# kohonda/mppi_playground

Hardware: AMD Instinct MI355X
Metric: sample_steps_per_sec (higher is better)
Workload: dtype f32

## Files before the change

mppi_playground_amd/csrc/mppi_capi.hip:

```cpp
#include <hip/hip_runtime.h>
#include <dlfcn.h>
#include <rccl/rccl.h>

#include <cmath>
#include <cstdio>
#include <cstring>
#include <new>
#include <string>
#include <vector>

#include "../../include/mppi_hip.h"
#include "host_search.hpp"
#include "mppi_kernels.hpp"

using namespace mppi;

static constexpr int FOLD_IN_FINALIZE_MAX_ROWS = 64;

struct MppiSolver {
    MppiConfig cfg{};
    Dims d{};
    int ds = 0, dc = 0;
    float4* noise = nullptr;
    float* costs = nullptr;
    unsigned* min_key = nullptr;
    int min_slot = 0;
    float* x0 = nullptr;
    const float* x0_cur = nullptr;
    float* x0_used = nullptr;
    float* coltab = nullptr;
    bool wide = false, limits_set = true;
    mppi::host::MpoState* mpo_dev = nullptr;
// ... 84 lines not shown
    uint8_t* map_pad = nullptr;
    size_t map_bytes[2] = {0, 0}, map_pad_bytes = 0;
    bool params_set = false;
    ModelCtx ctx{};
    int math_fast = 2;
    int reduce_blocks = 512;
    int reduce_chains = 0;
    int timing = 0;
    std::vector<hipEvent_t> ev_pool[5];
    size_t ev_used[5] = {0, 0, 0, 0, 0};
    int GPW = 8, nchunks = 1, colsp = 128;
    bool summary_valid = false;
    int* live_hint = nullptr;
    int* live_hint_dev = nullptr;
    int fold_mode = 0;
    int lazy_state = 0;
    float* b1 = nullptr;
    float* pending_state_out = nullptr;
    uint32_t pending_serial = 0;
    hipStream_t pending_stream = nullptr;
    hipEvent_t lazy_ev = nullptr;
    uint32_t finalize_serial = 0;
    std::string err;
};

namespace {

int fail(mppi_handle_t h, int code, const std::string& msg) {
    if (h) h->err = msg;
    return code;
// ... 237 lines not shown
    d.row = d.T * md.dc;
    d.R = (d.row + 3) / 4;
    for (int k = 0; k < MPPI_MAX_DIM_CONTROL; ++k) {
        d.u_min[k] = cfg->u_min[k]; d.u_max[k] = cfg->u_max[k]; d.sigma[k] = cfg->sigmas[k];
    }
    h->wide = cfg->model == MPPI_MODEL_GENERIC && md.dc != 1 && md.dc != 2 && md.dc != 4;
    h->GPW = 8;
    const int chg = h->GPW * (BLOCK / WAVE);
    h->nchunks = (d.R + chg - 1) / chg;
    h->colsp = h->nchunks * chg * 4;
    *out = h;
    HIP_TRY(h, hipSetDevice(cfg->device));
    const size_t noise_bytes = (size_t)d.tiles * d.R * 64 * sizeof(float4);
    HIP_TRY(h, hipMalloc(&h->noise, noise_bytes));
    HIP_TRY(h, hipMemset(h->noise, 0, noise_bytes));
    HIP_TRY(h, hipMalloc(&h->costs, sizeof(float) * (size_t)d.N));
    HIP_TRY(h, hipMalloc(&h->min_key, 2 * sizeof(unsigned)));
    HIP_TRY(h, hipMemset(h->min_key, 0xFF, 2 * sizeof(unsigned)));
    const size_t x0_floats = (size_t)std::max(md.ds, MPPI_MAX_DIM_STATE);
    HIP_TRY(h, hipMalloc(&h->x0, sizeof(float) * x0_floats));
    HIP_TRY(h, hipMemset(h->x0, 0, sizeof(float) * x0_floats));
    h->x0_cur = h->x0;
    HIP_TRY(h, hipMalloc(&h->x0_used, sizeof(float) * x0_floats));
    HIP_TRY(h, hipMemset(h->x0_used, 0, sizeof(float) * x0_floats));
    h->gen = GenCtx{(uint32_t)cfg->seed, (uint32_t)(cfg->seed >> 32), 0u};
    d.dc = md.dc;
    HIP_TRY(h, hipMalloc(&h->mean, sizeof(float) * (size_t)d.row));
    HIP_TRY(h, hipMemset(h->mean, 0, sizeof(float) * (size_t)d.row));
    HIP_TRY(h, hipMalloc(&h->mean_used, sizeof(float) * (size_t)d.row));
    HIP_TRY(h, hipMemset(h->mean_used, 0, sizeof(float) * (size_t)d.row));
    HIP_TRY(h, hipMalloc(&h->solve_stats, sizeof(float) * 8));
// ... 133 lines not shown
    CLONE(summary, sizeof(float) * (size_t)(MPPI_SUMMARY_HEAD + d.row));
    CLONE(mpo_dev, sizeof(mppi::host::MpoState));
    CLONE(mpo_temp_dev, sizeof(float));
    CLONE(lbps_dev, sizeof(LbpsDev));
    CLONE(lams_dev, sizeof(float) * 3 * STATS_L);
    CLONE(essps_dev, sizeof(EsspsDev));
    CLONE(lambda_dev, sizeof(float));
    if (src->grid0_dev) {
        if (!dst->grid0_dev) HIP_TRY(dst, hipMalloc(&dst->grid0_dev, sizeof(double) * STATS_L));
        CLONE(grid0_dev, sizeof(double) * STATS_L);
    }
#undef CLONE
    dst->min_slot = src->min_slot; dst->gen = src->gen; dst->tiles_valid = src->tiles_valid; dst->injected = src->injected;
    dst->noise_regen = src->noise_regen; dst->mapping = src->mapping; dst->math_fast = src->math_fast;
    dst->reduce_blocks = src->reduce_blocks; dst->reduce_chains = src->reduce_chains; dst->fold_mode = src->fold_mode;
    dst->fused_mode = src->fused_mode; dst->fused_timeout_ticks = src->fused_timeout_ticks; dst->lbps_grid = src->lbps_grid;
    dst->essps_merge0 = src->essps_merge0;
    dst->auto_rule = src->auto_rule; dst->auto_param = src->auto_param; dst->auto_lo = src->auto_lo; dst->auto_hi = src->auto_hi;
    dst->lbps_lo = src->lbps_lo; dst->lbps_hi = src->lbps_hi; dst->grid0_lo = src->grid0_lo; dst->grid0_hi = src->grid0_hi;
    dst->essps_lo = src->essps_lo; dst->essps_hi = src->essps_hi; dst->essps_range = src->essps_range;
    dst->essps_prev_host = src->essps_prev_host; dst->essps_prev_lo = src->essps_prev_lo; dst->essps_prev_hi = src->essps_prev_hi;
    dst->lambda_dev_valid = src->lambda_dev_valid;
    for (int i = 0; i < 3; ++i) dst->stats_host[8 + STATS_L * 3 + i] = src->stats_host[8 + STATS_L * 3 + i];
    dst->last_reduce_blocks = 0;
    dst->summary_valid = src->summary_valid || src->last_reduce_blocks > 0;
    if (!src->summary_valid && src->last_reduce_blocks > 0) {
        if (int rc = clone_buf(dst, dst->partials, src->partials, sizeof(float) * (size_t)2048 * src->colsp)) return rc;
        if (int rc = clone_buf(dst, dst->heads, src->heads, sizeof(float) * (size_t)2048 * 4)) return rc;
        dst->last_reduce_blocks = src->last_reduce_blocks; dst->summary_valid = false;
    }
// ... 566 lines not shown
    const bool defer = h->lazy_state && state_out && !generic && h->mapping == 0;
    if (h->pending_state_out) { if (int rc = flush_state_seq(h, s)) return rc; }
    {
        StageTimer tm(h, 3, s);
#define CALL_FINALIZE(MODEL, FASTV)                                                                   \
    hipLaunchKernelGGL((finalize_kernel<MODEL, FASTV>), dim3(1), dim3(FIN_BLOCK), shmem, s, summaries_dev, num_shards, \
                       h->partials, h->heads, mk, h->last_reduce_blocks, h->colsp, h->summary, h->live_hint_dev,  \
                       lambda, lam_dev, h->d.row, h->d.T, h->x0_cur, store_mean ? h->mean : (float*)nullptr, action_out,  \
                       defer ? (float*)nullptr : state_out, stats_out, h->solve_stats, sg, p2p, h->ctx,          \
                       defer ? h->b1 : (float*)nullptr, defer ? state_out : (float*)nullptr)
        MPPI_DISPATCH(h, CALL_FINALIZE);
#undef CALL_FINALIZE
    }
    HIP_TRY(h, hipGetLastError());
    ++h->finalize_serial;
    if (defer) { h->pending_state_out = state_out; h->pending_serial = h->finalize_serial; h->pending_stream = s; }
    return MPPI_OK;
}

static int order_behind_pending(mppi_handle_t h, hipStream_t s) {
    if (s == h->pending_stream) return MPPI_OK;
    if (!h->lazy_ev) HIP_TRY(h, hipEventCreateWithFlags(&h->lazy_ev, hipEventDisableTiming));
    HIP_TRY(h, hipEventRecord(h->lazy_ev, h->pending_stream));
    HIP_TRY(h, hipStreamWaitEvent(s, h->lazy_ev, 0));
    return MPPI_OK;
}

static int flush_state_seq(mppi_handle_t h, hipStream_t s) {
    if (!h->pending_state_out) return MPPI_OK;
    float* out = h->pending_state_out;
// ... 132 lines not shown
    HIP_TRY(h, hipGetLastError());
    if (rule != FUSED_RULE_NONE) h->lambda_dev_valid = true;
    h->last_reduce_blocks = 0;
    h->summary_valid = true;
    return MPPI_OK;
}

int mppi_set_auto_lambda(mppi_handle_t h, int rule, double param, double lam_min, double lam_max) {
    if (!h || rule < MPPI_AUTO_NONE || rule > MPPI_AUTO_MPO) return fail(h, MPPI_E_INVALID, "bad temperature rule");
    if ((rule == MPPI_AUTO_ESSPS || rule == MPPI_AUTO_LBPS) && (!(lam_min > 0.0) || !(lam_max > lam_min) || !(param > 0.0)))
        return fail(h, MPPI_E_INVALID, "bad temperature rule arguments");
    h->auto_rule = rule; h->auto_param = param; h->auto_lo = lam_min; h->auto_hi = lam_max;
    return MPPI_OK;
}

int mppi_solve(mppi_handle_t h, const float* x0_dev, uint32_t solve_idx, float lambda, float* action_out_dev,
               float* state_seq_out_dev, float* stats_out_dev, void* stream) {
    if (!h) return MPPI_E_INVALID;
    const bool dev = lambda == MPPI_LAMBDA_DEVICE;
    if (dev && h->auto_rule == MPPI_AUTO_NONE)
        return fail(h, MPPI_E_STATE, "MPPI_LAMBDA_DEVICE: no temperature rule configured (mppi_set_auto_lambda)");
    if (x0_dev) { if (int rc = mppi_bind_state(h, x0_dev)) return rc; }
    if (int rc = mppi_sample(h, solve_idx, stream)) return rc;
    if (fused_applies(h, lambda)) {
        if (int rc = flush_state_seq(h, (hipStream_t)stream)) return rc;
        bool declined = false;
        if (int rc = solve_fused(h, lambda, action_out_dev, state_seq_out_dev, stats_out_dev, (hipStream_t)stream, &declined)) return rc;
        if (!declined) {
            if (h->auto_rule == MPPI_AUTO_MPO) return mppi_mpo_step_device(h, stream);
            return MPPI_OK;
        }
    }
    if (int rc = mppi_rollout_cost(h, stream)) return rc;
    if (dev && h->auto_rule == MPPI_AUTO_ESSPS) {
        if (int rc = mppi_essps_lambda_device(h, h->auto_param, h->auto_lo, h->auto_hi, stream)) return rc;
    } else if (dev && h->auto_rule == MPPI_AUTO_LBPS) {
        if (int rc = h->lbps_grid ? mppi_lbps_lambda_device(h, h->auto_param, h->auto_lo, h->auto_hi, stream)
                                  : mppi_lbps_brent_device(h, h->auto_param, h->auto_lo, h->auto_hi, stream)) return rc;
    }
    if (int rc = mppi_weights_reduce(h, lambda, nullptr, stream)) return rc;
    if (int rc = mppi_finalize(h, nullptr, 1, lambda, 1, action_out_dev, state_seq_out_dev, stats_out_dev, stream)) return rc;
    if (h->auto_rule == MPPI_AUTO_MPO) return mppi_mpo_step_device(h, stream);
    return MPPI_OK;
}

int mppi_set_sg_filter(mppi_handle_t h, const float* coeffs_host, int window, const float* history_host) {
// ... 635 lines not shown
        return MPPI_OK;
    }
    if (k == "fused_rearm") {
        if (h->fused_error) *(volatile int*)h->fused_error = 0;
        return MPPI_OK;
    }
    if (k == "lazy_state_seq") {
        if (value && !h->b1) HIP_TRY(h, hipMalloc(&h->b1, sizeof(float) * ((size_t)h->d.row + MPPI_MAX_DIM_STATE)));
        h->lazy_state = value ? 1 : 0;
        return MPPI_OK;
    }
    if (k == "lbps_search") { h->lbps_grid = value ? 1 : 0; return MPPI_OK; }
    if (k == "search_test_drop_block") { h->brent_drop_block = value ? 1 : 0; return MPPI_OK; }
    if (k == "search_rearm") { if (h->search_error) *(volatile int*)h->search_error = 0; return MPPI_OK; }
    if (k == "essps_merge0") { h->essps_merge0 = value != 0; return MPPI_OK; }
    if (k == "fold_path") { h->fold_mode = (value >= 0 && value <= 2) ? (int)value : 0; return MPPI_OK; }
    if (k == "exchange_p2p") {
        if (value && !h->p2p_connected) return fail(h, MPPI_E_STATE, "exchange_p2p: call mppi_p2p_alloc / mppi_p2p_connect first");
        h->p2p_enabled = value != 0;
        return MPPI_OK;
    }
    if (k == "exchange_comm") {
        if (value && !h->comm) return fail(h, MPPI_E_STATE, "exchange_comm: call mppi_comm_init first");
        h->comm_enabled = value != 0;
        return MPPI_OK;
    }
    if (k == "noise_regen") { h->noise_regen = value ? 1 : 0; h->tiles_valid = h->tiles_valid && h->injected; return MPPI_OK; }
    return fail(h, MPPI_E_INVALID, "unknown option " + k);
}

// ... 37 lines not shown
```

mppi_playground_amd/csrc/mppi_finalize.hpp:

```cpp
#pragma once
#include "mppi_exchange.hpp"
#include "mppi_reduce.hpp"

namespace mppi {

template <int NT>
__device__ __forceinline__ int compact_live_rows(const float* __restrict__ heads, int nblocks,
                                                 unsigned short* __restrict__ s_list, int* __restrict__ s_wcnt) {
    constexpr int NWV = NT / WAVE;
    constexpr int MAXCH = REDUCE_MAX_BLOCKS / NT;
    const int lane = threadIdx.x & 63, wv = threadIdx.x >> 6;
    const int nch = (nblocks + NT - 1) / NT;
    unsigned long long mine = 0ull;
    for (int ch = 0; ch < nch; ++ch) {
        const int bb = ch * NT + threadIdx.x;
        const bool f = bb < nblocks && heads[(int64_t)bb * 4 + 3] != 0.0f;
        const unsigned long long mask = __ballot(f);
        if (f) mine |= 1ull << ch;
        if (lane == 0) s_wcnt[ch * NWV + wv] = __popcll(mask);
    }
    __syncthreads();
    int nlive = 0;
    for (int ch = 0; ch < nch; ++ch) {
        int off = 0;
// ... 179 lines not shown
    }
    if (threadIdx.x == 0) rollout_states_checked<MODEL, FAST>(s_x0, T, ctx, state_out, getu);
}

template <int MODEL, int FAST>
__global__ __launch_bounds__(WAVE) void state_seq_kernel(const float* __restrict__ b1_in, int row, int T,
                                                         float* __restrict__ state_out, ModelCtx ctx) {
    constexpr int DS = ModelT<MODEL, FAST>::DS;
    extern __shared__ __attribute__((aligned(16))) float s_b1[];
    for (int i = threadIdx.x; i < row + DS; i += WAVE) s_b1[i] = b1_in[i];
    __syncthreads();
    batch1_rollout<MODEL, FAST>(ctx, s_b1 + row, s_b1, T, state_out);
}

constexpr int FIN_BLOCK = 1024;
template <int MODEL, int FAST>
__device__ __forceinline__ void finalize_tail(const float* summaries, int num_shards, float lambda, int row, int T,
                                              const float* s_x0, float* s_act, float* s_yp,
                                              float* __restrict__ mean_store, float* __restrict__ action_out,
                                              float* __restrict__ state_out, float* __restrict__ stats_out,
                                              float* __restrict__ stats_keep, const SgFilter& sg, const ModelCtx& ctx,
                                              float* __restrict__ b1_out = nullptr, float* __restrict__ poison_out = nullptr) {
    const int stride = MPPI_SUMMARY_HEAD + row;
    float xmax = -INFINITY, cmin = INFINITY;
    for (int g = 0; g < num_shards; ++g) {
        const float m = summaries[(int64_t)g * stride];
        xmax = fmaxf(xmax, (-m) / lambda);
        cmin = fminf(cmin, m);
    }
    float se = 0.f, se2 = 0.f, sec = 0.f;
    for (int g = 0; g < num_shards; ++g) {
        const float* sm = summaries + (int64_t)g * stride;
        const float f = expf((-sm[0]) / lambda - xmax);
        se = fmaf(f, sm[1], se);
        se2 = fmaf(f * f, sm[2], se2);
        sec = fmaf(f, sm[3], sec);
    }
    for (int cidx = threadIdx.x; cidx < row; cidx += FIN_BLOCK) {
        float a = 0.f;
        for (int g = 0; g < num_shards; ++g) {
            const float* sm = summaries + (int64_t)g * stride;
            const float f = expf((-sm[0]) / lambda - xmax);
            a = fmaf(f, sm[MPPI_SUMMARY_HEAD + cidx], a);
        }
        a = a / se;
        s_act[cidx] = a;
        if (sg.window == 0) {
            if (action_out) action_out[cidx] = a;
            if (mean_store) mean_store[cidx] = a;
        }
    }
    if (threadIdx.x == 0) {
        if (stats_out) { stats_out[0] = cmin; stats_out[1] = se; stats_out[2] = se2; stats_out[3] = sec; }
        stats_keep[0] = cmin; stats_keep[1] = se; stats_keep[2] = se2; stats_keep[3] = sec;
        stats_keep[4] = lambda;
    }
    __syncthreads();
    if (sg.window > 0) {
        const int dcn = row / T, p = sg.window / 2, n = 2 * T - 1;
        for (int idx = threadIdx.x; idx < n * dcn; idx += FIN_BLOCK) {
            const int i = idx / dcn, k = idx - i * dcn;
            s_yp[(p + i) * dcn + k] = i < T - 1 ? sg.history[i * dcn + k] : s_act[(i - (T - 1)) * dcn + k];
        }
        __syncthreads();
        for (int idx = threadIdx.x; idx < p * dcn; idx += FIN_BLOCK) {
            const int j = idx / dcn, k = idx - j * dcn;
            s_yp[(p - 1 - j) * dcn + k] = s_yp[(p + j) * dcn + k];
            s_yp[(p + n + j) * dcn + k] = s_yp[(p + n - 1 - j) * dcn + k];
        }
        __syncthreads();
        float filt = 0.0f;
        const int cidx = threadIdx.x;
        if (cidx < row) {
            const int t = cidx / dcn, k = cidx - t * dcn;
            for (int j = 0; j < sg.window; ++j) filt = filt + s_yp[(T - 1 + t + j) * dcn + k] * sg.coeffs[j];
        }
        __syncthreads();
        if (cidx < row) {
            s_act[cidx] = filt;
            if (action_out) action_out[cidx] = filt;
            if (mean_store) mean_store[cidx] = filt;
        }
        for (int idx = threadIdx.x; idx < (T - 1) * dcn; idx += FIN_BLOCK) {
            const int i = idx / dcn, k = idx - i * dcn;
            sg.history[idx] = i < T - 2 ? s_yp[(p + i + 1) * dcn + k] : 0.0f;
        }
        __syncthreads();
        if (threadIdx.x < dcn && T >= 2) sg.history[(T - 2) * dcn + threadIdx.x] = s_act[threadIdx.x];
        __syncthreads();
    }
    if (b1_out) {
        for (int cidx = threadIdx.x; cidx < row; cidx += FIN_BLOCK) b1_out[cidx] = s_act[cidx];
        if (threadIdx.x < ModelT<MODEL, FAST>::DS) b1_out[row + threadIdx.x] = s_x0[threadIdx.x];
        if (poison_out)
            for (int c = threadIdx.x; c < (T + 1) * ModelT<MODEL, FAST>::DS; c += FIN_BLOCK) poison_out[c] = __uint_as_float(0x7fc00000u);
    }
    if (!state_out) return;
    batch1_rollout<MODEL, FAST>(ctx, s_x0, s_act, T, state_out);
}

template <int MODEL, int FAST>
__global__ __launch_bounds__(FIN_BLOCK) void finalize_kernel(const float* __restrict__ summaries, int num_shards,
                                                             const float* __restrict__ partials,
                                                             const float* __restrict__ heads,
                                                             const unsigned* __restrict__ min_key, int nblocks,
                                                             int colsp, float* __restrict__ summary_out,
                                                             int* __restrict__ nlive_out, float lambda_arg,
                                                             const float* __restrict__ lambda_dev, int row, int T,
                                                             const float* __restrict__ x0,
                                                             float* __restrict__ mean_store,
// ... 80 lines not shown
```

mppi_playground_amd/csrc/mppi_kernels.hpp:

```cpp
#pragma once
#include "mppi_common.hpp"
#include "mppi_sample.hpp"
#include "mppi_rollout.hpp"
#include "mppi_reduce.hpp"
#include "mppi_exchange.hpp"
#include "mppi_finalize.hpp"
#include "mppi_search.hpp"
#include "mppi_fused.hpp"
#include "mppi_topk.hpp"
#include "mppi_env.hpp"
#include "mppi_layout.hpp"
#include "mppi_maps.hpp"
```

mppi_playground_amd/csrc/mppi_rollout.hpp:

```cpp
#pragma once
#include "mppi_sample.hpp"

namespace mppi {

template <int MODEL, int FAST, bool GEN, bool UC, bool VAR = false, bool X0OUT = false>
__device__ __forceinline__ float trajectory_cost(const float4* __restrict__ np, uint64_t gi, const GenCtx& gen,
                                                 const float4* mean4, const float* ktab,
                                                 const float* __restrict__ x0, const Dims& d, const ModelCtx& ctx_in,
                                                 bool& bad) {
    using M = ModelT<MODEL, FAST>;
    using K = typename M::K;
    constexpr int DS = M::DS, DC = M::DC, SPG = 4 / DC;
    ModelCtx ctx = ctx_in;
    if constexpr (FAST != 0 && EntryGeneral<M>::value) M::pin_hot(ctx);
    KeyPins pins{gen.seed_lo, gen.seed_hi, gen.seed_lo + 0x9E3779B9u};
    if (GEN) asm volatile("" : "+v"(pins.k0v), "+v"(pins.k1v), "+v"(pins.k0w));
    float s[DS], pu[DC], pl[DC];
#pragma unroll
    for (int j = 0; j < DS; ++j) s[j] = x0[j];
    if (FAST) {
        if constexpr (EntryGeneral<M>::value) {
            M::enter_any(s);
        } else {
            M::check_state(ctx, s, bad);
// ... 94 lines not shown
        if (bad) {
            bool ignore = false;
            total = trajectory_cost<MODEL, 0, GEN, false>(np, gi, gen, mp, s_ktab, x0, d, ctx, ignore);
        }
    }
    return total;
}

template <int MODEL, int FAST>
__device__ __forceinline__ void batch1_rollout(const ModelCtx& ctx, const float* s_x0, const float* s_act, int T,
                                               float* __restrict__ state_out);

#ifndef MPPI_ROLLOUT_ATTR
#define MPPI_ROLLOUT_ATTR
#endif
template <int MODEL, int FAST, bool GEN, bool UC>
__global__ __launch_bounds__(BLOCK) MPPI_ROLLOUT_ATTR void rollout_cost_kernel(const float4* __restrict__ noise,
                                                             const float* __restrict__ mean,
                                                             const float* __restrict__ x0,
                                                             float* __restrict__ costs,
                                                             unsigned* __restrict__ min_key,
                                                             unsigned* __restrict__ next_min_key,
                                                             float* __restrict__ mean_used,
                                                             float* __restrict__ x0_used, Dims d, GenCtx gen,
                                                             ModelCtx ctx, const float* __restrict__ b1_in,
                                                             float* __restrict__ b1_state_out) {
    using M = ModelT<MODEL, FAST>;
    __shared__ float s_min[BLOCK / WAVE];
    extern __shared__ __attribute__((aligned(16))) float s_dyn[];
    if (b1_state_out != nullptr && blockIdx.x == gridDim.x - 1) {
        for (int i = threadIdx.x; i < d.row + M::DS; i += BLOCK) s_dyn[i] = b1_in[i];
        __syncthreads();
        batch1_rollout<MODEL, FAST>(ctx, s_dyn + d.row, s_dyn, d.T, b1_state_out);
        return;
    }
#ifdef MPPI_AB_VGPR_FLOOR
    asm volatile("; vgpr floor" ::: "v84");
#endif
    if (blockIdx.x == 0 && threadIdx.x < M::DS) x0_used[threadIdx.x] = x0[threadIdx.x];
    float4* s_mean4 = reinterpret_cast<float4*>(s_dyn);
    float* s_ktab = s_dyn + 8 * d.R;
    for (int f = threadIdx.x; f < 4 * d.R; f += BLOCK) {
        const float m = f < d.row ? mean[f] : 0.0f;
        s_dyn[f] = m;
        s_dyn[4 * d.R + f] = 0.0f;
        if (blockIdx.x == 0 && f < d.row) mean_used[f] = m;
    }
    for (int f = threadIdx.x; f < d.T * M::KROW; f += BLOCK) s_ktab[f] = ctx.ref[f];
    __syncthreads();
    const int lane = threadIdx.x & 63, wid = threadIdx.x >> 6;
    const int64_t tile = (int64_t)blockIdx.x * (BLOCK / WAVE) + wid;
    if (blockIdx.x == 0 && threadIdx.x == 0) *next_min_key = 0xFFFFFFFFu;
    float total = INFINITY;
    if (tile < d.tiles) {
        const int64_t i = tile * 64 + lane;
        const uint64_t gi = (uint64_t)(d.sample_offset + i);
        const bool inherit = (d.sample_offset + i) < d.inherit_count;
        const float4* np = noise + tile * d.R * 64 + lane;
        bool bad = false;
        const float4* mp = inherit ? s_mean4 : s_mean4 + d.R;
        total = lane_cost<MODEL, FAST, GEN, UC>(np, gi, gen, mp, s_ktab, x0, d, ctx);
        if (i < d.N) costs[i] = total;
        else total = INFINITY;
    }
    const float wm = wave_min(total);
    if (lane == 0) s_min[wid] = wm;
    __syncthreads();
    if (threadIdx.x == 0) {
        float m = s_min[0];
#pragma unroll
        for (int w = 1; w < BLOCK / WAVE; ++w) m = fminf(m, s_min[w]);
        if (m < INFINITY) atomicMin(min_key, float_to_key(m));
    }
}

template <int MODEL, int FAST>
__global__ __launch_bounds__(BLOCK) void rollout_cost_wave_kernel(const float* __restrict__ eps_std,
                                                                  const float* __restrict__ mean,
                                                                  const float* __restrict__ x0,
                                                                  float* __restrict__ costs,
                                                                  unsigned* __restrict__ min_key,
                                                                  unsigned* __restrict__ next_min_key, Dims d,
                                                                  ModelCtx ctx) {
    using M = ModelT<MODEL, FAST>;
    using K = typename M::K;
    constexpr int DS = M::DS, DC = M::DC, NW = BLOCK / WAVE;
    extern __shared__ __attribute__((aligned(16))) float s_dyn[];
    const int lane = threadIdx.x & 63, wid = threadIdx.x >> 6;
// ... 53 lines not shown
```

Baseline: 364.5 billion.

## Add fused single-block tail kernel for sparse-live MPPI solves

Adds a new solve path for the case where few tiles carry non-negligible weight. The rollout kernel now also writes a per-tile minimum, and a single-block tail kernel then skips dead tiles, regenerates noise only for live tiles, accumulates the weighted partials, reduces them and runs finalize in the same block. This is meant to replace the separate reduce, summary and finalize launches and the full-width weighted reduction with one small kernel. The path is gated on a live-row hint from the previous solve, an occupancy check, LDS limits and various config conditions, and finalize_tail gains a thread-count template parameter so it can run at the smaller block size.

```diff
diff --git a/mppi_playground_amd/csrc/mppi_capi.hip b/mppi_playground_amd/csrc/mppi_capi.hip
--- a/mppi_playground_amd/csrc/mppi_capi.hip
+++ b/mppi_playground_amd/csrc/mppi_capi.hip
@@ -16,6 +16,7 @@
 using namespace mppi;
 
 static constexpr int FOLD_IN_FINALIZE_MAX_ROWS = 64;
+static constexpr int TAIL_MAX_LIVE_ROWS = 8;
 
 struct MppiSolver {
     MppiConfig cfg{};
@@ -130,6 +131,11 @@
     int* live_hint = nullptr;
     int* live_hint_dev = nullptr;
     int fold_mode = 0;
+    bool hint_seen = false;
+    int fused_tail = 1;
+    float* tile_min = nullptr;
+    int tail_occ_key = 0;
+    bool tail_occ_ok = false;
     int lazy_state = 0;
     float* b1 = nullptr;
     float* pending_state_out = nullptr;
@@ -397,7 +403,8 @@
     const size_t noise_bytes = (size_t)d.tiles * d.R * 64 * sizeof(float4);
     HIP_TRY(h, hipMalloc(&h->noise, noise_bytes));
     HIP_TRY(h, hipMemset(h->noise, 0, noise_bytes));
-    HIP_TRY(h, hipMalloc(&h->costs, sizeof(float) * (size_t)d.N));
+    HIP_TRY(h, hipMalloc(&h->costs, sizeof(float) * (size_t)d.tiles * 65));
+    h->tile_min = h->costs + d.tiles * 64;
     HIP_TRY(h, hipMalloc(&h->min_key, 2 * sizeof(unsigned)));
     HIP_TRY(h, hipMemset(h->min_key, 0xFF, 2 * sizeof(unsigned)));
     const size_t x0_floats = (size_t)std::max(md.ds, MPPI_MAX_DIM_STATE);
@@ -561,6 +568,8 @@
     dst->min_slot = src->min_slot; dst->gen = src->gen; dst->tiles_valid = src->tiles_valid; dst->injected = src->injected;
     dst->noise_regen = src->noise_regen; dst->mapping = src->mapping; dst->math_fast = src->math_fast;
     dst->reduce_blocks = src->reduce_blocks; dst->reduce_chains = src->reduce_chains; dst->fold_mode = src->fold_mode;
+    dst->fused_tail = src->fused_tail; dst->hint_seen = src->hint_seen;
+    *dst->live_hint = *(volatile int*)src->live_hint;
     dst->fused_mode = src->fused_mode; dst->fused_timeout_ticks = src->fused_timeout_ticks; dst->lbps_grid = src->lbps_grid;
     dst->essps_merge0 = src->essps_merge0;
     dst->auto_rule = src->auto_rule; dst->auto_param = src->auto_param; dst->auto_lo = src->auto_lo; dst->auto_hi = src->auto_hi;
@@ -1157,6 +1166,7 @@
     }
     HIP_TRY(h, hipGetLastError());
     ++h->finalize_serial;
+    if (!p2p.seq) h->hint_seen = true;
     if (defer) { h->pending_state_out = state_out; h->pending_serial = h->finalize_serial; h->pending_stream = s; }
     return MPPI_OK;
 }
@@ -1319,6 +1329,91 @@
     return MPPI_OK;
 }
 
+static int64_t reduce_grid(mppi_handle_t h) {
+    const int64_t blocks = std::min<int64_t>(h->reduce_blocks, (h->d.tiles + 3) / 4);
+    return std::max<int64_t>(1, std::min<int64_t>(blocks, REDUCE_MAX_BLOCKS));
+}
+static size_t tail_lds_bytes(mppi_handle_t h) {
+    return sizeof(float) * tail_lds_floats(h->d.R, h->d.row, h->d.T, h->dc, h->sg_window);
+}
+static bool tail_occupancy_ok(mppi_handle_t h) {
+    const int key = math_level(h) + 1;
+    if (h->tail_occ_key == key) return h->tail_occ_ok;
+    bool ok = false;
+#define CALL_OCC(MODEL, FASTV)                                                                        \
+    do {                                                                                              \
+        const size_t rsh = sizeof(float) * std::max((size_t)8 * h->d.R + (size_t)h->d.T * ModelT<MODEL, FASTV>::KROW, \
+                                                    (size_t)h->d.row + MPPI_MAX_DIM_STATE);           \
+        int plain = 0, tail = 0;                                                                      \
+        ok = hipOccupancyMaxActiveBlocksPerMultiprocessor(&plain, rollout_cost_kernel<MODEL, FASTV, true, FASTV != 0>, \
+                                                          BLOCK, rsh) == hipSuccess &&                \
+             hipOccupancyMaxActiveBlocksPerMultiprocessor(&tail, rollout_tail_pick<MODEL, FASTV>(), BLOCK, rsh) == hipSuccess && \
+             tail >= plain;                                                                           \
+    } while (0)
+    MPPI_DISPATCH(h, CALL_OCC);
+#undef CALL_OCC
+    h->tail_occ_key = key;
+    h->tail_occ_ok = ok;
+    return ok;
+}
+static bool tail_applies(mppi_handle_t h, float lambda) {
+    if (!h->fused_tail || h->cfg.model == MPPI_MODEL_GENERIC || h->mapping != 0) return false;
+    const bool dev = lambda == MPPI_LAMBDA_DEVICE;
+    if (dev && h->auto_rule != MPPI_AUTO_MPO) return false;
+    if (dev && !h->lambda_dev_valid) return false;
+    if (!dev && !(lambda > 0.0f)) return false;
+    if (!(h->noise_regen && !h->injected && !h->wide)) return false;
+    if (h->p2p_enabled || h->comm_enabled) return false;
+    if (h->lazy_state) return false;
+    if (h->timing == 1) return false;
+    if (h->nchunks != 1) return false;
+    if (h->d.tiles > (int64_t)TAIL_MAX_ROUNDS * reduce_grid(h) * 4 * 8) return false;
+    if (!h->hint_seen || *(volatile int*)h->live_hint > TAIL_MAX_LIVE_ROWS) return false;
+    if (tail_lds_bytes(h) > (size_t)48 * 1024) return false;
+    if (check_ready(h) != MPPI_OK) return false;
+    return tail_occupancy_ok(h);
+}
+
+static int solve_tail(mppi_handle_t h, float lambda, float* action_out, float* state_out, float* stats_out, hipStream_t s) {
+    const float* lam_dev = nullptr;
+    if (int rc = resolve_lambda(h, lambda, &lam_dev)) return rc;
+    const int64_t nvb = reduce_grid(h);
+    h->min_slot ^= 1;
+    unsigned* mk = h->min_key + h->min_slot;
+    unsigned* mk_next = h->min_key + (h->min_slot ^ 1);
+    TailArgs ta{};
+    ta.tile_min = h->tile_min;
+    ta.nvb = (int)nvb; ta.colsp = h->colsp; ta.partials = h->partials; ta.heads = h->heads;
+    ta.summary = h->summary; ta.nlive_out = h->live_hint_dev;
+    ta.lambda_arg = lambda; ta.lambda_dev = lam_dev; ta.mean = h->mean;
+    ta.mean_store = h->mean; ta.action_out = action_out; ta.state_out = state_out; ta.stats_out = stats_out;
+    ta.stats_keep = h->solve_stats;
+    ta.sg = SgFilter{h->sg_coeffs, h->sg_history, h->sg_window > 0 ? h->sg_window : 0};
+    const unsigned grid = (unsigned)((h->d.tiles + 3) / 4);
+    const size_t tail_sh = tail_lds_bytes(h);
+#define CALL_TAIL(MODEL, FASTV)                                                                       \
+    do {                                                                                              \
+        const size_t rsh = sizeof(float) * std::max((size_t)8 * h->d.R + (size_t)h->d.T * ModelT<MODEL, FASTV>::KROW, \
+                                                    (size_t)h->d.row + MPPI_MAX_DIM_STATE);           \
+        {                                                                                             \
+            StageTimer tm(h, 1, s);                                                                   \
+            hipLaunchKernelGGL((rollout_tail_pick<MODEL, FASTV>()), dim3(grid), dim3(BLOCK), rsh, s, h->noise, h->mean, \
+                               h->x0_cur, h->costs, mk, mk_next, h->mean_used, h->x0_used, h->d, h->gen, h->ctx, \
+                               (const float*)nullptr, (float*)nullptr);                               \
+        }                                                                                             \
+        hipLaunchKernelGGL((tail_kernel<MODEL, FASTV>), dim3(1), dim3(BLOCK), tail_sh, s, (const float*)h->costs, \
+                           (const unsigned*)mk, h->x0_cur, h->d, h->gen, h->ctx, ta);                 \
+    } while (0)
+    MPPI_DISPATCH(h, CALL_TAIL);
+#undef CALL_TAIL
+    HIP_TRY(h, hipGetLastError());
+    h->last_reduce_blocks = (int)nvb;
+    h->summary_valid = true;
+    h->hint_seen = true;
+    ++h->finalize_serial;
+    return MPPI_OK;
+}
+
 int mppi_solve(mppi_handle_t h, const float* x0_dev, uint32_t solve_idx, float lambda, float* action_out_dev,
                float* state_seq_out_dev, float* stats_out_dev, void* stream) {
     if (!h) return MPPI_E_INVALID;
@@ -1335,6 +1430,11 @@
             if (h->auto_rule == MPPI_AUTO_MPO) return mppi_mpo_step_device(h, stream);
             return MPPI_OK;
         }
+    }
+    if (tail_applies(h, lambda)) {
+        if (int rc = solve_tail(h, lambda, action_out_dev, state_seq_out_dev, stats_out_dev, (hipStream_t)stream)) return rc;
+        if (h->auto_rule == MPPI_AUTO_MPO) return mppi_mpo_step_device(h, stream);
+        return MPPI_OK;
     }
     if (int rc = mppi_rollout_cost(h, stream)) return rc;
     if (dev && h->auto_rule == MPPI_AUTO_ESSPS) {
@@ -2000,6 +2100,7 @@
     if (k == "search_test_drop_block") { h->brent_drop_block = value ? 1 : 0; return MPPI_OK; }
     if (k == "search_rearm") { if (h->search_error) *(volatile int*)h->search_error = 0; return MPPI_OK; }
     if (k == "essps_merge0") { h->essps_merge0 = value != 0; return MPPI_OK; }
+    if (k == "fused_tail") { h->fused_tail = value ? 1 : 0; return MPPI_OK; }
     if (k == "fold_path") { h->fold_mode = (value >= 0 && value <= 2) ? (int)value : 0; return MPPI_OK; }
     if (k == "exchange_p2p") {
         if (value && !h->p2p_connected) return fail(h, MPPI_E_STATE, "exchange_p2p: call mppi_p2p_alloc / mppi_p2p_connect first");
diff --git a/mppi_playground_amd/csrc/mppi_finalize.hpp b/mppi_playground_amd/csrc/mppi_finalize.hpp
--- a/mppi_playground_amd/csrc/mppi_finalize.hpp
+++ b/mppi_playground_amd/csrc/mppi_finalize.hpp
@@ -217,7 +217,7 @@
 }
 
 constexpr int FIN_BLOCK = 1024;
-template <int MODEL, int FAST>
+template <int MODEL, int FAST, int NT = FIN_BLOCK>
 __device__ __forceinline__ void finalize_tail(const float* summaries, int num_shards, float lambda, int row, int T,
                                               const float* s_x0, float* s_act, float* s_yp,
                                               float* __restrict__ mean_store, float* __restrict__ action_out,
@@ -239,7 +239,7 @@
         se2 = fmaf(f * f, sm[2], se2);
         sec = fmaf(f, sm[3], sec);
     }
-    for (int cidx = threadIdx.x; cidx < row; cidx += FIN_BLOCK) {
+    for (int cidx = threadIdx.x; cidx < row; cidx += NT) {
         float a = 0.f;
         for (int g = 0; g < num_shards; ++g) {
             const float* sm = summaries + (int64_t)g * stride;
@@ -261,30 +261,39 @@
     __syncthreads();
     if (sg.window > 0) {
         const int dcn = row / T, p = sg.window / 2, n = 2 * T - 1;
-        for (int idx = threadIdx.x; idx < n * dcn; idx += FIN_BLOCK) {
+        for (int idx = threadIdx.x; idx < n * dcn; idx += NT) {
             const int i = idx / dcn, k = idx - i * dcn;
             s_yp[(p + i) * dcn + k] = i < T - 1 ? sg.history[i * dcn + k] : s_act[(i - (T - 1)) * dcn + k];
         }
         __syncthreads();
-        for (int idx = threadIdx.x; idx < p * dcn; idx += FIN_BLOCK) {
+        for (int idx = threadIdx.x; idx < p * dcn; idx += NT) {
             const int j = idx / dcn, k = idx - j * dcn;
             s_yp[(p - 1 - j) * dcn + k] = s_yp[(p + j) * dcn + k];
             s_yp[(p + n + j) * dcn + k] = s_yp[(p + n - 1 - j) * dcn + k];
         }
         __syncthreads();
-        float filt = 0.0f;
-        const int cidx = threadIdx.x;
-        if (cidx < row) {
-            const int t = cidx / dcn, k = cidx - t * dcn;
-            for (int j = 0; j < sg.window; ++j) filt = filt + s_yp[(T - 1 + t + j) * dcn + k] * sg.coeffs[j];
-        }
-        __syncthreads();
-        if (cidx < row) {
-            s_act[cidx] = filt;
-            if (action_out) action_out[cidx] = filt;
-            if (mean_store) mean_store[cidx] = filt;
-        }
-        for (int idx = threadIdx.x; idx < (T - 1) * dcn; idx += FIN_BLOCK) {
+        constexpr int NV = FIN_BLOCK / NT;
+        float filt[NV];
+#pragma unroll
+        for (int v = 0; v < NV; ++v) {
+            filt[v] = 0.0f;
+            const int cidx = threadIdx.x + v * NT;
+            if (cidx < row) {
+                const int t = cidx / dcn, k = cidx - t * dcn;
+                for (int j = 0; j < sg.window; ++j) filt[v] = filt[v] + s_yp[(T - 1 + t + j) * dcn + k] * sg.coeffs[j];
+            }
+        }
+        __syncthreads();
+#pragma unroll
+        for (int v = 0; v < NV; ++v) {
+            const int cidx = threadIdx.x + v * NT;
+            if (cidx < row) {
+                s_act[cidx] = filt[v];
+                if (action_out) action_out[cidx] = filt[v];
+                if (mean_store) mean_store[cidx] = filt[v];
+            }
+        }
+        for (int idx = threadIdx.x; idx < (T - 1) * dcn; idx += NT) {
             const int i = idx / dcn, k = idx - i * dcn;
             sg.history[idx] = i < T - 2 ? s_yp[(p + i + 1) * dcn + k] : 0.0f;
         }
@@ -293,10 +302,10 @@
         __syncthreads();
     }
     if (b1_out) {
-        for (int cidx = threadIdx.x; cidx < row; cidx += FIN_BLOCK) b1_out[cidx] = s_act[cidx];
+        for (int cidx = threadIdx.x; cidx < row; cidx += NT) b1_out[cidx] = s_act[cidx];
         if (threadIdx.x < ModelT<MODEL, FAST>::DS) b1_out[row + threadIdx.x] = s_x0[threadIdx.x];
         if (poison_out)
-            for (int c = threadIdx.x; c < (T + 1) * ModelT<MODEL, FAST>::DS; c += FIN_BLOCK) poison_out[c] = __uint_as_float(0x7fc00000u);
+            for (int c = threadIdx.x; c < (T + 1) * ModelT<MODEL, FAST>::DS; c += NT) poison_out[c] = __uint_as_float(0x7fc00000u);
     }
     if (!state_out) return;
     batch1_rollout<MODEL, FAST>(ctx, s_x0, s_act, T, state_out);
diff --git a/mppi_playground_amd/csrc/mppi_kernels.hpp b/mppi_playground_amd/csrc/mppi_kernels.hpp
--- a/mppi_playground_amd/csrc/mppi_kernels.hpp
+++ b/mppi_playground_amd/csrc/mppi_kernels.hpp
@@ -11,3 +11,4 @@
 #include "mppi_env.hpp"
 #include "mppi_layout.hpp"
 #include "mppi_maps.hpp"
+#include "mppi_tail.hpp"
diff --git a/mppi_playground_amd/csrc/mppi_rollout.hpp b/mppi_playground_amd/csrc/mppi_rollout.hpp
--- a/mppi_playground_amd/csrc/mppi_rollout.hpp
+++ b/mppi_playground_amd/csrc/mppi_rollout.hpp
@@ -132,6 +132,66 @@
 #ifndef MPPI_ROLLOUT_ATTR
 #define MPPI_ROLLOUT_ATTR
 #endif
+template <int MODEL, int FAST, bool GEN, bool UC, bool TAIL>
+__device__ __forceinline__ void rollout_cost_body(const float4* __restrict__ noise, const float* __restrict__ mean,
+                                                  const float* __restrict__ x0, float* __restrict__ costs,
+                                                  unsigned* __restrict__ min_key, unsigned* __restrict__ next_min_key,
+                                                  float* __restrict__ mean_used, float* __restrict__ x0_used, const Dims& d,
+                                                  const GenCtx& gen, const ModelCtx& ctx, const float* __restrict__ b1_in,
+                                                  float* __restrict__ b1_state_out, float* s_dyn) {
+    using M = ModelT<MODEL, FAST>;
+    __shared__ float s_min[BLOCK / WAVE];
+    if (!TAIL && b1_state_out != nullptr && blockIdx.x == gridDim.x - 1) {
+        for (int i = threadIdx.x; i < d.row + M::DS; i += BLOCK) s_dyn[i] = b1_in[i];
+        __syncthreads();
+        batch1_rollout<MODEL, FAST>(ctx, s_dyn + d.row, s_dyn, d.T, b1_state_out);
+        return;
+    }
+#ifdef MPPI_AB_VGPR_FLOOR
+    asm volatile("; vgpr floor" ::: "v84");
+#endif
+    if (blockIdx.x == 0 && threadIdx.x < M::DS) x0_used[threadIdx.x] = x0[threadIdx.x];
+    float4* s_mean4 = reinterpret_cast<float4*>(s_dyn);
+    float* s_ktab = s_dyn + 8 * d.R;
+    for (int f = threadIdx.x; f < 4 * d.R; f += BLOCK) {
+        const float m = f < d.row ? mean[f] : 0.0f;
+        s_dyn[f] = m;
+        s_dyn[4 * d.R + f] = 0.0f;
+        if (blockIdx.x == 0 && f < d.row) mean_used[f] = m;
+    }
+    for (int f = threadIdx.x; f < d.T * M::KROW; f += BLOCK) s_ktab[f] = ctx.ref[f];
+    __syncthreads();
+    const int lane = threadIdx.x & 63, wid = threadIdx.x >> 6;
+    const int64_t tile = (int64_t)blockIdx.x * (BLOCK / WAVE) + wid;
+    if (blockIdx.x == 0 && threadIdx.x == 0) *next_min_key = 0xFFFFFFFFu;
+    float total = INFINITY;
+    bool any_nan = false;
+    if (tile < d.tiles) {
+        const int64_t i = tile * 64 + lane;
+        const uint64_t gi = (uint64_t)(d.sample_offset + i);
+        const bool inherit = (d.sample_offset + i) < d.inherit_count;
+        const float4* np = noise + tile * d.R * 64 + lane;
+        bool bad = false;
+        const float4* mp = inherit ? s_mean4 : s_mean4 + d.R;
+        total = lane_cost<MODEL, FAST, GEN, UC>(np, gi, gen, mp, s_ktab, x0, d, ctx);
+        if (i < d.N) costs[i] = total;
+        else total = INFINITY;
+        if constexpr (TAIL) any_nan = __ballot(total != total) != 0ull;
+    }
+    const float wm = wave_min(total);
+    if constexpr (TAIL) {
+        if (tile < d.tiles && lane == 0) costs[d.tiles * 64 + tile] = any_nan ? __uint_as_float(0x7fc00000u) : wm;
+    }
+    if (lane == 0) s_min[wid] = wm;
+    __syncthreads();
+    if (threadIdx.x == 0) {
+        float m = s_min[0];
+#pragma unroll
+        for (int w = 1; w < BLOCK / WAVE; ++w) m = fminf(m, s_min[w]);
+        if (m < INFINITY) atomicMin(min_key, float_to_key(m));
+    }
+}
+
 template <int MODEL, int FAST, bool GEN, bool UC>
 __global__ __launch_bounds__(BLOCK) MPPI_ROLLOUT_ATTR void rollout_cost_kernel(const float4* __restrict__ noise,
                                                              const float* __restrict__ mean,
@@ -143,53 +203,9 @@
                                                              float* __restrict__ x0_used, Dims d, GenCtx gen,
                                                              ModelCtx ctx, const float* __restrict__ b1_in,
                                                              float* __restrict__ b1_state_out) {
-    using M = ModelT<MODEL, FAST>;
-    __shared__ float s_min[BLOCK / WAVE];
     extern __shared__ __attribute__((aligned(16))) float s_dyn[];
-    if (b1_state_out != nullptr && blockIdx.x == gridDim.x - 1) {
-        for (int i = threadIdx.x; i < d.row + M::DS; i += BLOCK) s_dyn[i] = b1_in[i];
-        __syncthreads();
-        batch1_rollout<MODEL, FAST>(ctx, s_dyn + d.row, s_dyn, d.T, b1_state_out);
-        return;
-    }
-#ifdef MPPI_AB_VGPR_FLOOR
-    asm volatile("; vgpr floor" ::: "v84");
-#endif
-    if (blockIdx.x == 0 && threadIdx.x < M::DS) x0_used[threadIdx.x] = x0[threadIdx.x];
-    float4* s_mean4 = reinterpret_cast<float4*>(s_dyn);
-    float* s_ktab = s_dyn + 8 * d.R;
-    for (int f = threadIdx.x; f < 4 * d.R; f += BLOCK) {
-        const float m = f < d.row ? mean[f] : 0.0f;
-        s_dyn[f] = m;
-        s_dyn[4 * d.R + f] = 0.0f;
-        if (blockIdx.x == 0 && f < d.row) mean_used[f] = m;
-    }
-    for (int f = threadIdx.x; f < d.T * M::KROW; f += BLOCK) s_ktab[f] = ctx.ref[f];
-    __syncthreads();
-    const int lane = threadIdx.x & 63, wid = threadIdx.x >> 6;
-    const int64_t tile = (int64_t)blockIdx.x * (BLOCK / WAVE) + wid;
-    if (blockIdx.x == 0 && threadIdx.x == 0) *next_min_key = 0xFFFFFFFFu;
-    float total = INFINITY;
-    if (tile < d.tiles) {
-        const int64_t i = tile * 64 + lane;
-        const uint64_t gi = (uint64_t)(d.sample_offset + i);
-        const bool inherit = (d.sample_offset + i) < d.inherit_count;
-        const float4* np = noise + tile * d.R * 64 + lane;
-        bool bad = false;
-        const float4* mp = inherit ? s_mean4 : s_mean4 + d.R;
-        total = lane_cost<MODEL, FAST, GEN, UC>(np, gi, gen, mp, s_ktab, x0, d, ctx);
-        if (i < d.N) costs[i] = total;
-        else total = INFINITY;
-    }
-    const float wm = wave_min(total);
-    if (lane == 0) s_min[wid] = wm;
-    __syncthreads();
-    if (threadIdx.x == 0) {
-        float m = s_min[0];
-#pragma unroll
-        for (int w = 1; w < BLOCK / WAVE; ++w) m = fminf(m, s_min[w]);
-        if (m < INFINITY) atomicMin(min_key, float_to_key(m));
-    }
+    rollout_cost_body<MODEL, FAST, GEN, UC, false>(noise, mean, x0, costs, min_key, next_min_key, mean_used, x0_used, d,
+                                                     gen, ctx, b1_in, b1_state_out, s_dyn);
 }
 
 template <int MODEL, int FAST>
diff --git a/mppi_playground_amd/csrc/mppi_tail.hpp b/mppi_playground_amd/csrc/mppi_tail.hpp
--- /dev/null
+++ b/mppi_playground_amd/csrc/mppi_tail.hpp
@@ -0,0 +1,316 @@
+#pragma once
+#include "mppi_finalize.hpp"
+#include "mppi_rollout.hpp"
+
+namespace mppi {
+
+constexpr int TAIL_MAX_ROUNDS = 4;
+constexpr float TAIL_DEAD_ARG = -110.0f;
+
+struct TailArgs {
+    const float* tile_min;
+    int nvb, colsp;
+    float* partials;
+    float* heads;
+    float* summary;
+    int* nlive_out;
+    float lambda_arg;
+    const float* lambda_dev;
+    const float* mean;
+    float *mean_store, *action_out, *state_out, *stats_out, *stats_keep;
+    SgFilter sg;
+};
+
+__host__ __device__ inline size_t tail_lds_floats(int R, int row, int T, int dc, int sg_window) {
+    const size_t red = (size_t)(BLOCK / WAVE) * 8 * (WAVE + 1);
+    const size_t fin = (size_t)(MPPI_SUMMARY_HEAD + row) + row + (sg_window ? (size_t)(2 * T - 1 + 2 * (sg_window / 2)) * dc : 0);
+    return (size_t)8 * R + REDUCE_MAX_BLOCKS / 2 + (red > fin ? red : fin);
+}
+
+__device__ __forceinline__ bool tail_candidate(float m, float lambda, float xmax) {
+    return !((-m) / lambda - xmax <= TAIL_DEAD_ARG);
+}
+
+template <int MODEL, int FAST>
+__device__ __forceinline__ void solve_tail_block(float* s_dyn, const float* __restrict__ costs, const unsigned* __restrict__ min_key,
+                                                 const float* __restrict__ x0, const Dims& d, const GenCtx& gen,
+                                                 const ModelCtx& ctx, const TailArgs& ta) {
+    constexpr int NW = BLOCK / WAVE, TPW = 8, RP = 8, GPW = 8, NACC = GPW * 4;
+    __shared__ unsigned s_cand[REDUCE_MAX_BLOCKS / 32];
+    __shared__ unsigned s_live[TAIL_MAX_ROUNDS][NW];
+    __shared__ float s_head[NW][4];
+    __shared__ float s_x[NW][4];
+    __shared__ int s_n[2];
+    __shared__ float s_x0[MPPI_MAX_DIM_STATE];
+    const int lane = threadIdx.x & 63;
+    const int wid = __builtin_amdgcn_readfirstlane(threadIdx.x >> 6);
+    const float lambda = ta.lambda_dev ? *ta.lambda_dev : ta.lambda_arg;
+    const unsigned key = *min_key;
+    const float cmin = key_to_float(key);
+    const float xmax = (-cmin) / lambda;
+    const float4* s_mean4 = reinterpret_cast<const float4*>(s_dyn);
+    unsigned short* s_list = reinterpret_cast<unsigned short*>(s_dyn + 8 * d.R);
+    float* s_work = s_dyn + 8 * d.R + REDUCE_MAX_BLOCKS / 2;
+    float (*s_red)[RP][WAVE + 1] = reinterpret_cast<float (*)[RP][WAVE + 1]>(s_work);
+    const int nvb = ta.nvb;
+    const int64_t nwv = (int64_t)nvb * NW;
+    if (threadIdx.x < ModelT<MODEL, FAST>::DS) s_x0[threadIdx.x] = x0[threadIdx.x];
+    for (int w = threadIdx.x; w < REDUCE_MAX_BLOCKS / 32; w += BLOCK) s_cand[w] = 0u;
+    __syncthreads();
+    const auto mark = [&](int64_t t) {
+        const int vb = (int)((t % nwv) / NW);
+        atomicOr(&s_cand[vb >> 5], 1u << (vb & 31));
+    };
+    {
+        constexpr int U = 8;
+        const float4* tm4 = reinterpret_cast<const float4*>(ta.tile_min);
+        const int64_t n4 = d.tiles / 4;
+        for (int64_t base = 0; base < n4; base += (int64_t)U * BLOCK) {
+            float4 v[U];
+#pragma unroll
+            for (int u = 0; u < U; ++u) {
+                const int64_t j = base + u * BLOCK + threadIdx.x;
+                v[u] = j < n4 ? tm4[j] : make_float4(INFINITY, INFINITY, INFINITY, INFINITY);
+            }
+#pragma unroll
+            for (int u = 0; u < U; ++u) {
+                const int64_t j = base + u * BLOCK + threadIdx.x;
+                if (tail_candidate(v[u].x, lambda, xmax)) mark(4 * j);
+                if (tail_candidate(v[u].y, lambda, xmax)) mark(4 * j + 1);
+                if (tail_candidate(v[u].z, lambda, xmax)) mark(4 * j + 2);
+                if (tail_candidate(v[u].w, lambda, xmax)) mark(4 * j + 3);
+            }
+        }
+        for (int64_t t = 4 * n4 + threadIdx.x; t < d.tiles; t += BLOCK)
+            if (tail_candidate(ta.tile_min[t], lambda, xmax)) mark(t);
+    }
+    __syncthreads();
+    if (threadIdx.x == 0) {
+        int n = 0;
+        for (int w = 0; w < (nvb + 31) / 32; ++w)
+            for (unsigned b = s_cand[w]; b; b &= b - 1u) s_list[n++] = (unsigned short)(32 * w + __builtin_ctz(b));
+        s_n[0] = n;
+        s_n[1] = 0;
+    }
+    __syncthreads();
+    const int ncand = s_n[0];
+    const int ng = d.R;
+    const int full = ng / NW, rem = ng - full * NW;
+    const int nrounds = (int)((d.tiles + nwv * TPW - 1) / (nwv * TPW));
+    const auto lane_sum8 = [&](const float* a8) {
+#pragma unroll
+        for (int j = 0; j < RP; ++j) s_red[wid][j][lane] = a8[j];
+        __builtin_amdgcn_wave_barrier();
+        const float* rowp = &s_red[wid][lane & (RP - 1)][(lane >> 3) * 8];
+        float v0 = rowp[0] + rowp[1], v1 = rowp[2] + rowp[3], v2 = rowp[4] + rowp[5], v3 = rowp[6] + rowp[7];
+        float v = (v0 + v1) + (v2 + v3);
+        v += __shfl_xor(v, 8);
+        v += __shfl_xor(v, 16);
+        v += __shfl_xor(v, 32);
+        __builtin_amdgcn_wave_barrier();
+        return v;
+    };
+    for (int c = 0; c < ncand; ++c) {
+        const int vb = s_list[c];
+        float se = 0.0f, se2 = 0.0f, sec = 0.0f;
+        for (int rr = 0; rr < nrounds; ++rr) {
+            const int64_t base0 = (int64_t)vb * NW + (int64_t)rr * nwv * TPW;
+            unsigned live = 0, cand = 0;
+            float cq[TPW];
+#pragma unroll
+            for (int q = 0; q < TPW; ++q) {
+                const int64_t tile = base0 + wid + q * nwv;
+                cq[q] = tile < d.tiles ? ta.tile_min[tile] : INFINITY;
+            }
+#pragma unroll
+            for (int q = 0; q < TPW; ++q) cand |= (tail_candidate(cq[q], lambda, xmax) ? 1u : 0u) << q;
+#pragma unroll
+            for (int q = 0; q < TPW; ++q) {
+                const int64_t i = (base0 + wid + q * nwv) * 64 + lane;
+                cq[q] = ((cand >> q) & 1u) && i < d.N ? costs[i] : INFINITY;
+            }
+            for (int q = 0; q < TPW; ++q) {
+                if (!((cand >> q) & 1u)) continue;
+                const float cc = cq[q];
+                const float e = expf((-cc) / lambda - xmax);
+                const bool tile_live = __ballot(e != 0.0f) != 0ull;
+                live |= (tile_live ? 1u : 0u) << q;
+                if (tile_live) {
+                    const float cv = e != 0.0f ? cc : 0.0f;
+                    se += e;
+                    se2 = fmaf(e, e, se2);
+                    sec = fmaf(e, cv, sec);
+                }
+            }
+            if (lane == 0) s_live[rr][wid] = live;
+        }
+        __syncthreads();
+        bool block_live = false;
+        for (int rr = 0; rr < nrounds; ++rr)
+            for (int w2 = 0; w2 < NW; ++w2) block_live |= s_live[rr][w2] != 0u;
+        if (!block_live) {
+            __syncthreads();
+            continue;
+        }
+        const auto for_live_tiles = [&](auto&& body) {
+            for (int rr = 0; rr < nrounds; ++rr) {
+                const int64_t base0 = (int64_t)vb * NW + (int64_t)rr * nwv * TPW;
+                for (int w2 = 0; w2 < NW; ++w2) {
+                    const unsigned lv = __builtin_amdgcn_readfirstlane(s_live[rr][w2]);
+                    for (int q = 0; q < TPW; ++q) {
+                        if (!((lv >> q) & 1u)) continue;
+                        const int64_t tile = base0 + w2 + q * nwv;
+                        const int64_t i = tile * 64 + lane;
+                        const float cc = (i < d.N) ? costs[i] : INFINITY;
+                        const float e = expf((-cc) / lambda - xmax);
+                        const uint64_t gi = (uint64_t)(d.sample_offset + i);
+                        const bool inherit = (d.sample_offset + i) < d.inherit_count;
+                        body(tile, e, gi, inherit ? s_mean4 : s_mean4 + d.R);
+                    }
+                }
+            }
+        };
+        const auto accumulate4 = [&](float* a4, int g, const float4& n4, float e, const float4* mp) {
+            const float4 m4 = mp[g];
+            const float nv[4] = {n4.x, n4.y, n4.z, n4.w};
+            const float mv[4] = {m4.x, m4.y, m4.z, m4.w};
+#pragma unroll
+            for (int j = 0; j < 4; ++j) {
+                const int k = ctrl_index(j, d.dc);
+                const float u = clampf(mv[j] + nv[j], d.u_min[k], d.u_max[k]);
+                a4[j] = fmaf(e, u, a4[j]);
+            }
+        };
+        float* prow = ta.partials + (int64_t)vb * ta.colsp;
+        for (int p = 0; p < NACC / RP; ++p) {
+            if (2 * p >= full) break;
+            float acc8[RP];
+#pragma unroll
+            for (int j = 0; j < RP; ++j) acc8[j] = 0.0f;
+            for_live_tiles([&](int64_t, float e, uint64_t gi, const float4* mp) {
+#pragma unroll
+                for (int k = 0; k < 2; ++k) {
+                    const int m = 2 * p + k;
+                    if (m < full) accumulate4(&acc8[4 * k], wid + NW * m, noise_group<true>(nullptr, wid + NW * m, gi, gen, d), e, mp);
+                }
+            });
+            const float v = lane_sum8(acc8);
+            const int a = p * RP + lane;
+            if (lane < RP && (a >> 2) < full) prow[4 * (wid + NW * (a >> 2)) + (a & 3)] = v;
+        }
+        if (rem) {
+            float accx[4] = {0.0f, 0.0f, 0.0f, 0.0f};
+            for_live_tiles([&](int64_t tile, float e, uint64_t gi, const float4* mp) {
+                const bool mine = rem == 1 ? ((int)tile & 3) == wid : rem == 2 ? ((int)tile & 1) == (wid >> 1) : wid < rem;
+                if (mine) {
+                    const int g = NW * full + (rem == 1 ? 0 : rem == 2 ? (wid & 1) : wid);
+                    accumulate4(accx, g, noise_group<true>(nullptr, g, gi, gen, d), e, mp);
+                }
+            });
+            float x8[RP];
+#pragma unroll
+            for (int j = 0; j < RP; ++j) x8[j] = j < 4 ? accx[j & 3] : 0.0f;
+            const float v = lane_sum8(x8);
+            if (lane < 4) s_x[wid][lane] = v;
+            __syncthreads();
+            if (threadIdx.x < 4 * rem) {
+                const int j = threadIdx.x >> 2, jj = threadIdx.x & 3;
+                float t = 0.0f;
+#pragma unroll
+                for (int w = 0; w < NW; ++w)
+                    if (rem == 1 || (rem == 2 ? (w & 1) == j : w == j)) t += s_x[w][jj];
+                prow[4 * (NW * full + j) + jj] = t;
+            }
+        }
+        se = wave_sum(se);
+        se2 = wave_sum(se2);
+        sec = wave_sum(sec);
+        if (lane == 0) { s_head[wid][0] = se; s_head[wid][1] = se2; s_head[wid][2] = sec; }
+        __syncthreads();
+        if (threadIdx.x < 4) {
+            float v = 1.0f;
+            if (threadIdx.x < 3) {
+                v = 0.0f;
+#pragma unroll
+                for (int w = 0; w < NW; ++w) v += s_head[w][threadIdx.x];
+            }
+            ta.heads[(int64_t)vb * 4 + threadIdx.x] = v;
+        }
+        if (threadIdx.x == 0) s_list[s_n[1]++] = (unsigned short)vb;
+        __syncthreads();
+    }
+    const int nlive = s_n[1];
+    const int row = d.row;
+    float* s_sum = s_work;
+    float* s_act = s_sum + MPPI_SUMMARY_HEAD + row;
+    float* s_yp = s_act + row;
+    {
+        constexpr int NG = SUM_BLOCK / SUM_COLS;
+        const int ngr = min(NG, nlive);
+        for (int col = threadIdx.x; col < row + 3; col += BLOCK) {
+            const bool is_head = col >= row;
+            const float* base = is_head ? ta.heads + (col - row) : ta.partials + col;
+            const int64_t ld = is_head ? 4 : ta.colsp;
+            float v = 0.f;
+            for (int g = 0; g < ngr; ++g) {
+                float a[8];
+#pragma unroll
+                for (int q = 0; q < 8; ++q) a[q] = 0.f;
+                for (int k = g; k < nlive; k += 8 * NG) {
+#pragma unroll
+                    for (int q = 0; q < 8; ++q) {
+                        const int kk = k + q * NG;
+                        if (kk < nlive) a[q] += base[(int64_t)s_list[kk] * ld];
+                    }
+                }
+                v += ((a[0] + a[1]) + (a[2] + a[3])) + ((a[4] + a[5]) + (a[6] + a[7]));
+            }
+            const int dst = col < row ? MPPI_SUMMARY_HEAD + col : 1 + (col - row);
+            s_sum[dst] = v;
+            ta.summary[dst] = v;
+        }
+        if (threadIdx.x == 0) {
+            s_sum[0] = cmin;
+            ta.summary[0] = cmin;
+            *ta.nlive_out = nlive;
+        }
+    }
+    __syncthreads();
+    finalize_tail<MODEL, FAST, BLOCK>(s_sum, 1, lambda, row, d.T, s_x0, s_act, s_yp, ta.mean_store, ta.action_out, ta.state_out,
+                                      ta.stats_out, ta.stats_keep, ta.sg, ctx);
+}
+
+#define MPPI_ROLLOUT_TAIL_KERNEL(NAME, ATTR)                                                                          \
+    template <int MODEL, int FAST>                                                                                    \
+    __global__ __launch_bounds__(BLOCK) ATTR void NAME(                                                                \
+        const float4* __restrict__ noise, const float* __restrict__ mean, const float* __restrict__ x0,               \
+        float* __restrict__ costs, unsigned* __restrict__ min_key, unsigned* __restrict__ next_min_key,               \
+        float* __restrict__ mean_used, float* __restrict__ x0_used, Dims d, GenCtx gen, ModelCtx ctx,                 \
+        const float* __restrict__ b1_in, float* __restrict__ b1_state_out) {                                          \
+        extern __shared__ __attribute__((aligned(16))) float s_dyn[];                                                 \
+        rollout_cost_body<MODEL, FAST, true, FAST != 0, true>(noise, mean, x0, costs, min_key, next_min_key,          \
+                                                              mean_used, x0_used, d, gen, ctx, b1_in, b1_state_out, s_dyn); \
+    }
+MPPI_ROLLOUT_TAIL_KERNEL(rollout_tail_kernel, MPPI_ROLLOUT_ATTR)
+MPPI_ROLLOUT_TAIL_KERNEL(rollout_tail_kernel_w8, __attribute__((amdgpu_waves_per_eu(8))))
+#undef MPPI_ROLLOUT_TAIL_KERNEL
+template <int MODEL, int FAST>
+constexpr auto rollout_tail_pick() {
+    if constexpr (MODEL == MPPI_MODEL_RACING && FAST != 0) return &rollout_tail_kernel_w8<MODEL, FAST>;
+    else return &rollout_tail_kernel<MODEL, FAST>;
+}
+
+template <int MODEL, int FAST>
+__global__ __launch_bounds__(BLOCK) void tail_kernel(const float* __restrict__ costs, const unsigned* __restrict__ min_key,
+                                                     const float* __restrict__ x0, Dims d, GenCtx gen, ModelCtx ctx,
+                                                     TailArgs ta) {
+    extern __shared__ __attribute__((aligned(16))) float s_dyn[];
+    for (int f = threadIdx.x; f < 4 * d.R; f += BLOCK) {
+        s_dyn[f] = f < d.row ? ta.mean[f] : 0.0f;
+        s_dyn[4 * d.R + f] = 0.0f;
+    }
+    __syncthreads();
+    solve_tail_block<MODEL, FAST>(s_dyn, costs, min_key, x0, d, gen, ctx, ta);
+}
+
+}
```

New measurement: 309.0 billion (median of 2 runs). -15.2%, worse.
